# TomasDelaney/A-Deep-Reinforcement-Learning-Enabled-Soft-Exoskeleton-for-Parkinson-s-Patients

Measured on AMD Instinct MI355X. Metric: env steps/sec (batched exo sim) + TD7 grad-steps/sec at 1/2/4/8 MI355X, higher is better.
Workload: dtype f64 sim + bf16 TD7

## Files before the change

### a-deep-reinforcement-learning-enabled-soft-exoskeleton-for-parkinson-s-patients_amd/csrc/lap.hip

```cpp
#include <hip/hip_runtime.h>

#include <algorithm>
#include <cstdint>
#include <cstdlib>
#include <string>

#include "philox.h"
#include "exo_amd.h"

namespace {

constexpr int UPD_THREADS = 1024;

__device__ __forceinline__ float *stratum_tree(float *tree, int s, int cap) { return tree + (size_t)s * 2 * cap; }

constexpr int TOPN = 8192;
template <int NTOP = TOPN>
__device__ bool propagate_top(float *T, int cap, int levels, const int32_t *slot, int n, float *top) {
    int lv = 1;
    for (; lv <= levels && ((2 * cap) >> lv) > NTOP / 2; ++lv) {
        __syncthreads();
        for (int k = threadIdx.x; k < n; k += blockDim.x) {
            const int node = (cap + slot[k]) >> lv;
            T[node] = T[2 * node] + T[2 * node + 1];
        }
    }
    __syncthreads();
    if (lv > levels) return false;
    const int lim = min(NTOP, 2 * cap);
    if (blockDim.x == UPD_THREADS) {
        constexpr int PER = NTOP / UPD_THREADS;
        float v[PER];
#pragma unroll
        for (int j = 0; j < PER; ++j) {
            const int i = threadIdx.x + j * UPD_THREADS;
            v[j] = i < lim ? T[i] : 0.0f;
        }
#pragma unroll
        for (int j = 0; j < PER; ++j) {
            const int i = threadIdx.x + j * UPD_THREADS;
            if (i < lim) top[i] = v[j];
        }
    } else {
        for (int i = threadIdx.x; i < lim; i += blockDim.x) top[i] = T[i];
    }
    for (; lv <= levels; ++lv) {
        __syncthreads();
        for (int k = threadIdx.x; k < n; k += blockDim.x) {
            const int node = (cap + slot[k]) >> lv;
            top[node] = top[2 * node] + top[2 * node + 1];
        }
    }
    __syncthreads();
    const int wb = min(NTOP / 2, cap);
    for (int i = 1 + threadIdx.x; i < wb; i += blockDim.x) T[i] = top[i];
    __syncthreads();
    return true;
}
__device__ void propagate(float *T, int cap, int levels, const int32_t *slot, int n) {
    __shared__ float top[TOPN];
    propagate_top(T, cap, levels, slot, n, top);
}

__device__ void propagate_span(float *T, int cap, int levels, int capacity, int first, int count) {
    __shared__ float top[TOPN];
    if (count <= 0) return;
    int a0 = first, e0 = first + count, a1 = 0, e1 = 0;
    if (count >= capacity) {
        a0 = 0;
        e0 = capacity;
    } else if (e0 > capacity) {
        e1 = e0 - capacity;
        e0 = capacity;
    }
    int lv = 1;
    for (; lv <= levels && ((2 * cap) >> lv) > TOPN / 2; ++lv) {
        __syncthreads();
        const int lo0 = (cap + a0) >> lv, n0 = ((cap + e0 - 1) >> lv) - lo0 + 1;
        const int lo1 = (cap + a1) >> lv, n1 = e1 > a1 ? ((cap + e1 - 1) >> lv) - lo1 + 1 : 0;
        for (int k = threadIdx.x; k < n0 + n1; k += blockDim.x) {
            const int node = k < n0 ? lo0 + k : lo1 + k - n0;
            T[node] = T[2 * node] + T[2 * node + 1];
        }
    }
    __syncthreads();
    if (lv > levels) return;
    const int lim = min(TOPN, 2 * cap);
    for (int i = threadIdx.x; i < lim; i += blockDim.x) top[i] = T[i];
    for (; lv <= levels; ++lv) {
        __syncthreads();
        const int lo0 = (cap + a0) >> lv, n0 = ((cap + e0 - 1) >> lv) - lo0 + 1;
        const int lo1 = (cap + a1) >> lv, n1 = e1 > a1 ? ((cap + e1 - 1) >> lv) - lo1 + 1 : 0;
        for (int k = threadIdx.x; k < n0 + n1; k += blockDim.x) {
            const int node = k < n0 ? lo0 + k : lo1 + k - n0;
            top[node] = top[2 * node] + top[2 * node + 1];
        }
    }
    __syncthreads();
    const int wb = min(TOPN / 2, cap);
    for (int i = 1 + threadIdx.x; i < wb; i += blockDim.x) T[i] = top[i];
    __syncthreads();
}

constexpr int SPAN_LDS = 4096;
constexpr int SPAN_LEVELS = 32;
__device__ bool propagate_span_lds(float *T, int cap, int levels, int capacity, int first, int count,
                                   float *buf , float *edge ) {
    const int a = cap + first, e = cap + first + count - 1;
    if (count <= 0 || first + count > capacity || count > SPAN_LDS - 2 || levels >= SPAN_LEVELS) return false;
    const int t = threadIdx.x;
    if (t < 2 * levels) {
        const int lv = t >> 1, right = t & 1;
        const int lo = a >> lv, hi = e >> lv;
        if (!right && (lo & 1)) edge[t] = T[lo - 1];
        if (right && !(hi & 1)) edge[t] = T[hi + 1];
    }
    float *A = buf, *B = buf + SPAN_LDS;
    {
        const int base = a & ~1;
        for (int c = a + t; c <= e; c += blockDim.x) A[c - base] = T[c];
    }
    __syncthreads();
    if (t == 0) {
        if (a & 1) A[0] = edge[0];
        if (!(e & 1)) A[(e | 1) - (a & ~1)] = edge[1];
    }
    for (int lv = 1; lv <= levels; ++lv) {
        __syncthreads();
        const int lo = a >> lv, hi = e >> lv, cbase = (a >> (lv - 1)) & ~1, nbase = lo & ~1;
        for (int node = lo + t; node <= hi; node += blockDim.x) {
            const int c = 2 * node - cbase;
            const float v = A[c] + A[c + 1];
            T[node] = v;
            B[node - nbase] = v;
        }
        if (t == 0 && lv < levels) {
            if (lo & 1) B[0] = edge[2 * lv];
            if (!(hi & 1)) B[(hi | 1) - nbase] = edge[2 * lv + 1];
        }
        float *tmp = A;
        A = B;
        B = tmp;
    }
    __syncthreads();
    return true;
}

constexpr int ADD_CHUNK = 4096;
__global__ __launch_bounds__(UPD_THREADS) void lap_add_kernel(float *tree, const float *maxp, int cap, int levels,
                                                              int capacity, const int32_t *stratum,
                                                              const int32_t *slot, int n) {
    const int s = blockIdx.x;
    float *T = stratum_tree(tree, s, cap);
    __shared__ int32_t mine[ADD_CHUNK];
    __shared__ int count;
    const float p = *maxp;
    for (int base = 0; base < n; base += ADD_CHUNK) {
        if (threadIdx.x == 0) count = 0;
        __syncthreads();
// ... 845 lines not shown
}

__global__ __launch_bounds__(256) void lap_ref_plan_slots_kernel(int32_t *plan, long long entries,
                                                                 const int32_t *add_s, long long total,
                                                                 const long long *ref, int E, int capacity) {
    const long long i = (long long)blockIdx.x * blockDim.x + threadIdx.x;
    if (i >= entries) return;
    const int c = plan[i];
    if (c < 0) return;
    const long long ptr0 = ref[0], count0 = ref[1];
    const long long m0 = mult_below(count0, E), mr = mult_below(count0 + c, E);
    const long long qend = min(mr * E - count0, total - 1);
    const int s = add_s[c];
    bool win = true;
    for (long long q = c + 1; q <= qend; ++q) win &= add_s[q] != s;
    long long v = ptr0 + (mr - m0);
    if (v >= capacity) v -= capacity;
    if (v >= capacity) v %= capacity;
    plan[i] = win ? (int32_t)v : -1;
}

__global__ __launch_bounds__(256) void lap_ref_step_kernel(lap_storage_desc st, const int32_t *plan, int rows, int n,
                                                           long long *kk, int par, long long *k_dev,
                                                           const int32_t *strata, int capacity, const float *state,
                                                           const float *action, const float *next_state,
                                                           const float *reward, const uint8_t *done,
                                                           float action_scale, const uint8_t *table,
                                                           uint8_t *active, int32_t *count,
                                                           const int32_t *counts_table, double *score) {
    const long long k = kk[par];
    const long long k1 = k + 1 < rows ? k + 1 : rows - 1;
    const int e = blockIdx.x * 4 + (threadIdx.x >> 6), lane = threadIdx.x & 63;
    if (blockIdx.x == 0 && threadIdx.x == 0) {
        kk[par ^ 1] = k1;
        if (k_dev) *k_dev = k1;
        if (count) *count = counts_table[k1];
    }
    if (e >= n) return;
    const int slot = k < rows ? plan[(size_t)k * n + e] : -1;
    if (slot >= 0) {
        const long r = (long)strata[e] * (capacity + 1) + slot;
        const int sd = st.state_dim, ad = st.action_dim;
        for (int q = lane; q < sd; q += 64) {
            st.state[r * sd + q] = state[(long)e * sd + q];
            st.next_state[r * sd + q] = next_state[(long)e * sd + q];
        }
        for (int q = lane; q < ad; q += 64) st.action[r * ad + q] = action[(long)e * ad + q] / action_scale;
        if (lane == 0) {
            st.reward[r] = reward[e];
            st.not_done[r] = 1.0f - (done[e] ? 1.0f : 0.0f);
        }
    }
    if (lane == 0) {
        if (score) score[e] += active[e] ? (double)reward[e] : 0.0;
        active[e] = table[(size_t)k1 * n + e];
    }
}

__global__ __launch_bounds__(256) void lap_ref_commit_leaves_kernel(const int32_t *plan, long long entries, int n,
                                                                    const int32_t *strata, float *tree, int cap,
                                                                    const float *maxp) {
    const long long i = (long long)blockIdx.x * blockDim.x + threadIdx.x;
    if (i >= entries) return;
    const int slot = plan[i];
    if (slot < 0) return;
    stratum_tree(tree, strata[i % n], cap)[cap + slot] = *maxp;
}

__global__ __launch_bounds__(UPD_THREADS) void lap_ref_commit_tree_kernel(float *tree, int cap, int levels,
                                                                          int capacity, const long long *ref,
                                                                          long long total, int E) {
    const long long ptr0 = ref[0], count0 = ref[1];
    if (total <= 0) return;
    const long long last = mult_below(count0 + total - 1, E) - mult_below(count0, E);
    propagate_span(stratum_tree(tree, blockIdx.x, cap), cap, levels, capacity, (int)ptr0,
                   (int)min(last + 1, (long long)capacity));
}

__global__ void lap_ref_commit_ref_kernel(long long *ref, long long total, int E, int capacity, int32_t *ring_size) {
    const long long ptr0 = ref[0], count0 = ref[1], size0 = ref[2];
    const long long adv = mult_below(count0 + total, E) - mult_below(count0, E);
    const long long size = min(size0 + adv, (long long)capacity);
    for (int s = 0; s < E; ++s) ring_size[s] = (int32_t)size;
    ref[0] = (ptr0 + adv) % capacity;
    ref[1] = count0 + total;
    ref[2] = size;
}

constexpr int GATHER_DRAWS = 16;
__global__ __launch_bounds__(256) void lap_gather_kernel(lap_storage_desc st, int capacity, const int32_t *idx,
                                                         int batch, int total, float *o_state, float *o_action,
                                                         float *o_next, float *o_reward, float *o_not_done) {
    const int sd = st.state_dim, ad = st.action_dim;
    const bool v4 = (sd & 3) == 0 && ((reinterpret_cast<uintptr_t>(st.state) | reinterpret_cast<uintptr_t>(st.next_state) |
                                       reinterpret_cast<uintptr_t>(o_state) | reinterpret_cast<uintptr_t>(o_next)) & 15) == 0;
    const int sv = v4 ? sd / 4 : sd, per = 2 * sv + ad + 2;
    const int d0 = blockIdx.x * GATHER_DRAWS;
    const int nd = min(GATHER_DRAWS, total - d0);
    const int items = nd * per;
    constexpr int GU = 4;
    for (int it0 = threadIdx.x; it0 < items; it0 += GU * 256) {
        float4 v[GU];
        float *dst[GU];
        bool wide[GU];
#pragma unroll
        for (int u = 0; u < GU; ++u) {
            const int it = it0 + u * 256;
            dst[u] = nullptr;
            wide[u] = false;
            if (it >= items) continue;
            const int q = it / per, c = it - q * per;
            const long d = d0 + q;
            const long row = (long)(d / batch) * (capacity + 1) + idx[d];
            if (c < 2 * sv) {
                const bool nx = c >= sv;
                const int e = nx ? c - sv : c;
                const float *src = (nx ? st.next_state : st.state) + row * sd;
                float *o = (nx ? o_next : o_state) + d * sd;
                if (v4) {
                    v[u] = ld4(src + 4 * e);
                    dst[u] = o + 4 * e;
                    wide[u] = true;
                } else {
                    v[u].x = src[e];
                    dst[u] = o + e;
                }
            } else if (c < 2 * sv + ad) {
                const int e = c - 2 * sv;
                v[u].x = st.action[row * ad + e];
                dst[u] = o_action + d * ad + e;
            } else if (c == 2 * sv + ad) {
                v[u].x = st.reward[row];
                dst[u] = o_reward + d;
            } else {
                v[u].x = st.not_done[row];
                dst[u] = o_not_done + d;
            }
        }
#pragma unroll
        for (int u = 0; u < GU; ++u) {
            if (!dst[u]) continue;
            if (wide[u]) st4(dst[u], v[u]);
            else *dst[u] = v[u].x;
        }
    }
}

struct TdPrio {
    const float *td;
    float alpha, minp;
    float *out;
};

__global__ __launch_bounds__(UPD_THREADS) void lap_update_sample_kernel(float *tree, float *maxp, int cap, int levels,
                                                                        int capacity, const int32_t *idx_in,
                                                                        const float *prio, int batch,
                                                                        const int32_t *size, lap_storage_desc st,
                                                                        SampleRng rng, int32_t *idx_out,
                                                                        float *o_state, float *o_action, float *o_next,
                                                                        float *o_reward, float *o_not_done,
                                                                        TdPrio tp, bool gather) {
    const int s = blockIdx.x;
    float *T = stratum_tree(tree, s, cap);
    const int32_t *I = idx_in + (size_t)s * batch;
    const float *P = prio + (size_t)s * batch;
    __shared__ float red[UPD_THREADS / 64];
    __shared__ int32_t li[UPD_THREADS];
    __shared__ float top[TOPN_US];
    __shared__ int32_t pick[UPD_THREADS];
    const unsigned long long call = *rng.counter;
    float mx = 0.0f;
    for (int b0 = 0; b0 < batch; b0 += UPD_THREADS) {
        const int nb = min(UPD_THREADS, batch - b0);
        __syncthreads();
        if ((int)threadIdx.x < nb) li[threadIdx.x] = I[b0 + threadIdx.x];
        __syncthreads();
        const int b = b0 + threadIdx.x;
        if (b < batch) {
            const int me = li[threadIdx.x];
            bool last = true;
            for (int k = threadIdx.x + 1; k < nb; ++k) last &= (li[k] != me);
            for (int b2 = b0 + nb; b2 < batch; ++b2) last &= (I[b2] != me);
            float pb;
            if (tp.td) {
                const long d = (long)s * batch + b;
                pb = powf(fmaxf(fmaxf(tp.td[2 * d], tp.td[2 * d + 1]), tp.minp), tp.alpha);
                if (tp.out) tp.out[d] = pb;
            } else {
                pb = P[b];
            }
            if (last) T[cap + me] = pb;
            mx = fmaxf(mx, pb);
        }
    }
    for (int o = 32; o > 0; o >>= 1) mx = fmaxf(mx, __shfl_xor(mx, o, 64));
    if ((threadIdx.x & 63) == 0) red[threadIdx.x >> 6] = mx;
    const bool staged = propagate_top<TOPN_US>(T, cap, levels, I, batch, top);
    if (threadIdx.x == 0) {
        for (int w = 1; w < (int)(blockDim.x >> 6); ++w) mx = fmaxf(mx, red[w]);
        atomicMax(reinterpret_cast<int *>(maxp), __float_as_int(mx));
    }
    const int lim = staged ? min(TOPN_US, 2 * cap) : 0;
    auto node_at = [&](int node) { return node < lim ? top[node] : T[node]; };
    const int sz = size[s];
    const float tot = prefix_sum(node_at, cap, levels, sz);
    for (int b = threadIdx.x; b < batch; b += UPD_THREADS) {
        const int d = s * batch + b;
        uint32_t r[4];
        philox_block(rng.seed, rng.tag, call, (uint32_t)d, r);
        float val = u01_open_hi(r[0]) * tot;
        int node = 1, lv = 0;
        for (; lv < levels && 2 * node + 1 < lim; ++lv) {
            const float left = top[2 * node], right = top[2 * node + 1];
            if (val <= left || right <= 0.0f) {
                node = 2 * node;
            } else {
                val -= left;
                node = 2 * node + 1;
            }
        }
        node = descend_from([T](int n) { return T[n]; }, val, node, lv, levels);
        int i = node - cap;
        if (i >= sz) i = sz > 0 ? sz - 1 : 0;
        idx_out[d] = i;
        if (b < UPD_THREADS) pick[b] = i;
    }
    __syncthreads();
    if (!gather) {
        if (threadIdx.x == 0 && atomicAdd(rng.ticket, 1u) == gridDim.x - 1) {
            *rng.counter = call + 1ull;
            *rng.ticket = 0u;
        }
        return;
    }
    const int sd = st.state_dim, ad = st.action_dim;
    const bool v4 = (sd & 3) == 0 && ((reinterpret_cast<uintptr_t>(st.state) | reinterpret_cast<uintptr_t>(st.next_state) |
                                       reinterpret_cast<uintptr_t>(o_state) | reinterpret_cast<uintptr_t>(o_next)) & 15) == 0;
    const int sv = v4 ? sd / 4 : sd, per = 2 * sv + ad + 2;
    const int items = min(batch, UPD_THREADS) * per;
    constexpr int GU = 8;
    for (int it0 = threadIdx.x; it0 < items; it0 += GU * UPD_THREADS) {
        float4 v[GU];
        float *dst[GU];
        bool wide[GU];
#pragma unroll
        for (int u = 0; u < GU; ++u) {
            const int it = it0 + u * UPD_THREADS;
            dst[u] = nullptr;
            wide[u] = false;
            if (it >= items) continue;
            const int b = it / per, c = it - b * per;
            const long d = (long)s * batch + b;
            const long row = (long)s * (capacity + 1) + pick[b];
            if (c < 2 * sv) {
                const bool nx = c >= sv;
                const int e = nx ? c - sv : c;
                const float *src = (nx ? st.next_state : st.state) + row * sd;
                float *o = (nx ? o_next : o_state) + d * sd;
                if (v4) {
                    v[u] = ld4(src + 4 * e);
                    dst[u] = o + 4 * e;
                    wide[u] = true;
                } else {
                    v[u].x = src[e];
                    dst[u] = o + e;
                }
            } else if (c < 2 * sv + ad) {
                const int e = c - 2 * sv;
                v[u].x = st.action[row * ad + e];
                dst[u] = o_action + d * ad + e;
            } else if (c == 2 * sv + ad) {
                v[u].x = st.reward[row];
                dst[u] = o_reward + d;
            } else {
                v[u].x = st.not_done[row];
                dst[u] = o_not_done + d;
            }
        }
#pragma unroll
        for (int u = 0; u < GU; ++u) {
            if (!dst[u]) continue;
            if (wide[u]) st4(dst[u], v[u]);
            else *dst[u] = v[u].x;
        }
    }
    __syncthreads();
    if (threadIdx.x == 0) {
        if (atomicAdd(rng.ticket, 1u) == gridDim.x - 1) {
            *rng.counter = call + 1ull;
            *rng.ticket = 0u;
        }
    }
}

int rc(hipError_t e) { return e == hipSuccess ? EXO_OK : EXO_EDEVICE; }

int levels_of(const lap_tree_desc *t) {
    int lv = 0;
    while ((1 << lv) < t->cap) ++lv;
    return lv;
}

bool gather_split() {
    static const bool on = [] {
        const char *e = getenv("EXO_LAP_GATHER_SPLIT");
        return !(e && e[0] == '0');
    }();
    return on;
}

int gather_after(const lap_tree_desc *t, const lap_storage_desc *st, int batch, const int32_t *idx, float *o_state,
                 float *o_action, float *o_next, float *o_reward, float *o_not_done, void *stream) {
    if (hipGetLastError() != hipSuccess) return EXO_EDEVICE;
    if (!gather_split()) return EXO_OK;
    const int total = t->n_strata * batch;
    hipLaunchKernelGGL(lap_gather_kernel, dim3((total + GATHER_DRAWS - 1) / GATHER_DRAWS), dim3(256), 0,
                       (hipStream_t)stream, *st, t->capacity, idx, batch, total, o_state, o_action, o_next, o_reward,
                       o_not_done);
    return hipGetLastError() == hipSuccess ? EXO_OK : EXO_EDEVICE;
}

bool valid(const lap_tree_desc *t) {
    return t && t->tree && t->max_priority && t->n_strata > 0 && t->capacity > 0 && t->cap >= t->capacity &&
           (t->cap & (t->cap - 1)) == 0 && t->cap <= (1 << MAXLV);
}

}

extern "C" {

int32_t lap_tree_floats(int32_t n_strata, int32_t capacity) {
    int cap = 1;
    while (cap < capacity) cap <<= 1;
    return n_strata * 2 * cap;
}

int lap_init(const lap_tree_desc *t, void *stream) {
    if (!valid(t)) return EXO_EINVAL;
    hipError_t e = hipMemsetAsync(t->tree, 0, (size_t)t->n_strata * 2 * t->cap * sizeof(float), (hipStream_t)stream);
    if (e != hipSuccess) return EXO_EDEVICE;
    hipLaunchKernelGGL(lap_init_kernel, dim3(1), dim3(1), 0, (hipStream_t)stream, t->max_priority);
    return rc(hipGetLastError());
}

int lap_add(const lap_tree_desc *t, const int32_t *stratum, const int32_t *slot, int32_t n, void *stream) {
    if (!valid(t) || !stratum || !slot || n < 0) return EXO_EINVAL;
    if (n == 0) return EXO_OK;
    hipLaunchKernelGGL(lap_add_kernel, dim3(t->n_strata), dim3(UPD_THREADS), 0, (hipStream_t)stream, t->tree,
                       t->max_priority, t->cap, levels_of(t), t->capacity, stratum, slot, n);
    return rc(hipGetLastError());
}

int lap_sample(const lap_tree_desc *t, const float *u, const int32_t *size, int32_t batch, int32_t *idx, void *stream) {
    if (!valid(t) || !u || !size || !idx || batch <= 0) return EXO_EINVAL;
    const int th = 128;
    hipLaunchKernelGGL(lap_sample_kernel, dim3((batch + th - 1) / th, t->n_strata), dim3(th), 0, (hipStream_t)stream,
                       t->tree, t->cap, levels_of(t), u, size, batch, idx);
    return rc(hipGetLastError());
}

int lap_update(const lap_tree_desc *t, const int32_t *idx, const float *prio, int32_t batch, void *stream) {
    if (!valid(t) || !idx || !prio || batch <= 0) return EXO_EINVAL;
    hipLaunchKernelGGL(lap_update_kernel, dim3(t->n_strata), dim3(UPD_THREADS), 0, (hipStream_t)stream, t->tree,
                       t->max_priority, t->cap, levels_of(t), idx, prio, batch);
    return rc(hipGetLastError());
}

int lap_reset_max(const lap_tree_desc *t, void *stream) {
    if (!valid(t)) return EXO_EINVAL;
    hipError_t e = hipMemsetAsync(t->max_priority, 0, sizeof(float), (hipStream_t)stream);
    if (e != hipSuccess) return EXO_EDEVICE;
    hipLaunchKernelGGL(lap_reset_max_kernel, dim3(256), dim3(1024), 0, (hipStream_t)stream, t->tree, t->max_priority,
                       t->cap, t->n_strata);
    return rc(hipGetLastError());
}

int lap_totals(const lap_tree_desc *t, float *out, void *stream) {
    if (!valid(t) || !out) return EXO_EINVAL;
    hipLaunchKernelGGL(lap_totals_kernel, dim3((t->n_strata + 63) / 64), dim3(64), 0, (hipStream_t)stream, t->tree,
                       t->cap, t->n_strata, out);
    return rc(hipGetLastError());
}

int lap_store_batch(const lap_tree_desc *t, const lap_storage_desc *st, const float *state, const float *action,
                    const float *next_state, const float *reward, const uint8_t *done, const int32_t *strata,
                    const uint8_t *active, float action_scale, int32_t n, int32_t *row_ws, void *stream) {
    if (!valid(t) || !st || !st->state || !st->action || !st->next_state || !st->reward || !st->not_done ||
        !st->ptr || !st->size || st->state_dim <= 0 || st->action_dim <= 0 || !state || !action || !next_state ||
        !reward || !done || !strata || !row_ws || n < 0 || action_scale == 0.0f)
        return EXO_EINVAL;
    if (n == 0) return EXO_OK;
    const char *fused_var = getenv("EXO_LAP_STORE_FUSED");
    const bool fused_env = fused_var && fused_var[0] == '1';
    if (fused_env && n <= STORE_FUSED_MAX && n <= t->capacity) {
        const bool vec = (st->state_dim & 3) == 0 &&
                         ((reinterpret_cast<uintptr_t>(state) | reinterpret_cast<uintptr_t>(next_state) |
                           reinterpret_cast<uintptr_t>(st->state) | reinterpret_cast<uintptr_t>(st->next_state)) &
                          15) == 0;
        if (vec)
            hipLaunchKernelGGL(lap_store_fused_kernel<true>, dim3(t->n_strata), dim3(UPD_THREADS), 0,
                               (hipStream_t)stream, t->tree, t->max_priority, t->cap, levels_of(t), t->capacity,
                               st->ptr, st->size, strata, active, n, row_ws, *st, state, action, next_state, reward,
                               done, action_scale);
        else
            hipLaunchKernelGGL(lap_store_fused_kernel<false>, dim3(t->n_strata), dim3(UPD_THREADS), 0,
                               (hipStream_t)stream, t->tree, t->max_priority, t->cap, levels_of(t), t->capacity,
                               st->ptr, st->size, strata, active, n, row_ws, *st, state, action, next_state, reward,
                               done, action_scale);
        return rc(hipGetLastError());
    }
    if (n > 4 * STORE_CHUNK)
        hipLaunchKernelGGL(lap_store_rank_kernel<16>, dim3(t->n_strata), dim3(UPD_THREADS), 0, (hipStream_t)stream,
                           t->tree, t->max_priority, t->cap, levels_of(t), t->capacity, st->ptr, st->size, strata,
                           active, n, row_ws);
    else
        hipLaunchKernelGGL(lap_store_rank_kernel<4>, dim3(t->n_strata), dim3(UPD_THREADS), 0, (hipStream_t)stream,
                           t->tree, t->max_priority, t->cap, levels_of(t), t->capacity, st->ptr, st->size, strata,
                           active, n, row_ws);
    if (hipGetLastError() != hipSuccess) return EXO_EDEVICE;
    hipLaunchKernelGGL(lap_store_copy_kernel, dim3((n + 3) / 4), dim3(256), 0, (hipStream_t)stream, *st, state,
                       action, next_state, reward, done, action_scale, n, row_ws);
    return rc(hipGetLastError());
}

int lap_store_batch_ref(const lap_tree_desc *t, const lap_storage_desc *st, int64_t *ref_dev, const float *state,
                        const float *action, const float *next_state, const float *reward, const uint8_t *done,
                        const int32_t *strata, const uint8_t *active, float action_scale, int32_t n,
                        int32_t *ws_dev, void *stream) {
    if (!valid(t) || !st || !st->state || !st->action || !st->next_state || !st->reward || !st->not_done ||
        !st->size || st->state_dim <= 0 || st->action_dim <= 0 || !ref_dev || !state || !action || !next_state ||
        !reward || !done || !strata || !ws_dev || n < 0 || action_scale == 0.0f)
        return EXO_EINVAL;
    if (n == 0) return EXO_OK;
    int32_t *rank_row = ws_dev, *slot_of = ws_dev + n, *row_of = ws_dev + 2 * n;
    hipLaunchKernelGGL(lap_store_ref_slots_kernel, dim3(1), dim3(UPD_THREADS), 0, (hipStream_t)stream, t->capacity,
                       t->n_strata, (long long *)ref_dev, st->size, strata, active, n, rank_row, slot_of, row_of);
    if (hipGetLastError() != hipSuccess) return EXO_EDEVICE;
    hipLaunchKernelGGL(lap_add_kernel, dim3(t->n_strata), dim3(UPD_THREADS), 0, (hipStream_t)stream, t->tree,
                       t->max_priority, t->cap, levels_of(t), t->capacity, strata, slot_of, n);
    if (hipGetLastError() != hipSuccess) return EXO_EDEVICE;
    hipLaunchKernelGGL(lap_store_copy_kernel, dim3((n + 3) / 4), dim3(256), 0, (hipStream_t)stream, *st, state,
                       action, next_state, reward, done, action_scale, n, row_of);
    return rc(hipGetLastError());
}

static int store_ref_fused(const lap_tree_desc *t, const lap_storage_desc *st, int64_t *ref_dev,
                           const float *state, const float *action, const float *next_state, const float *reward,
                           const uint8_t *done, const int32_t *strata, const uint8_t *active, float action_scale,
                           int32_t n, uint32_t *ticket_dev, const MaskAdvance &adv, void *stream) {
    if (!valid(t) || !st || !st->state || !st->action || !st->next_state || !st->reward || !st->not_done ||
        !st->size || st->state_dim <= 0 || st->action_dim <= 0 || !ref_dev || !state || !action || !next_state ||
        !reward || !done || !strata || !ticket_dev || n < 0 || action_scale == 0.0f)
        return EXO_EINVAL;
    if (n == 0) return EXO_OK;
    const int E = t->n_strata;
    const int K = 1 + std::max(1, std::min(15, (n + E * 64 - 1) / (E * 64)));
    auto al16 = [](const void *p) { return ((uintptr_t)p & 15u) == 0; };
    const bool vec = st->state_dim % 4 == 0 && al16(state) && al16(next_state) && al16(st->state) &&
                     al16(st->next_state);
    if (vec)
        hipLaunchKernelGGL(lap_store_ref_fused_kernel<true>, dim3(E, K), dim3(UPD_THREADS), 0, (hipStream_t)stream,
                           t->tree, t->max_priority, t->cap, levels_of(t), t->capacity, E, (long long *)ref_dev,
                           st->size, *st, state, action, next_state, reward, done, action_scale, strata, active, n,
                           ticket_dev, adv);
    else
        hipLaunchKernelGGL(lap_store_ref_fused_kernel<false>, dim3(E, K), dim3(UPD_THREADS), 0, (hipStream_t)stream,
                           t->tree, t->max_priority, t->cap, levels_of(t), t->capacity, E, (long long *)ref_dev,
                           st->size, *st, state, action, next_state, reward, done, action_scale, strata, active, n,
                           ticket_dev, adv);
    return rc(hipGetLastError());
}

int lap_store_batch_ref_fused(const lap_tree_desc *t, const lap_storage_desc *st, int64_t *ref_dev,
                              const float *state, const float *action, const float *next_state, const float *reward,
                              const uint8_t *done, const int32_t *strata, const uint8_t *active, float action_scale,
                              int32_t n, uint32_t *ticket_dev, void *stream) {
    return store_ref_fused(t, st, ref_dev, state, action, next_state, reward, done, strata, active, action_scale, n,
                           ticket_dev, MaskAdvance{}, stream);
}

int lap_store_batch_ref_fused_adv(const lap_tree_desc *t, const lap_storage_desc *st, int64_t *ref_dev,
                                  const float *state, const float *action, const float *next_state,
                                  const float *reward, const uint8_t *done, const int32_t *strata, uint8_t *active,
                                  float action_scale, int32_t n, uint32_t *ticket_dev, const uint8_t *table,
                                  int32_t rows, int64_t *k_dev, int32_t *count_dev, double *score_dev, void *stream) {
    if (!table || rows <= 0 || !k_dev || !active) return EXO_EINVAL;
    return store_ref_fused(t, st, ref_dev, state, action, next_state, reward, done, strata, active, action_scale, n,
                           ticket_dev, MaskAdvance{table, rows, (long long *)k_dev, active, count_dev, score_dev},
                           stream);
}

int lap_sample_gather(const lap_tree_desc *t, const lap_storage_desc *st, const float *u, int32_t batch,
                      int32_t *idx, float *out_state, float *out_action, float *out_next_state, float *out_reward,
                      float *out_not_done, void *stream) {
    if (!valid(t) || !st || !st->size || !u || !idx || batch <= 0 || !out_state || !out_action ||
        !out_next_state || !out_reward || !out_not_done)
        return EXO_EINVAL;
    const int total = t->n_strata * batch;
    hipLaunchKernelGGL(lap_sample_gather_kernel, dim3((total + 3) / 4), dim3(256), 0, (hipStream_t)stream, t->tree,
                       t->cap, levels_of(t), t->capacity, u, st->size, batch, total, idx, *st, out_state, out_action,
                       out_next_state, out_reward, out_not_done, SampleRng{0, 0, nullptr, nullptr});
    return rc(hipGetLastError());
}

int lap_update_sample_rng(const lap_tree_desc *t, const lap_storage_desc *st, const int32_t *idx_in,
                          const float *prio, int32_t batch, uint64_t seed, uint32_t tag, unsigned long long *counter,
                          uint32_t *ticket, int32_t *idx_out, float *out_state, float *out_action,
                          float *out_next_state, float *out_reward, float *out_not_done, void *stream) {
    if (!valid(t) || !st || !st->size || !idx_in || !prio || !counter || !ticket || !idx_out || batch <= 0 ||
        batch > UPD_THREADS || !out_state || !out_action || !out_next_state || !out_reward || !out_not_done)
        return EXO_EINVAL;
    hipLaunchKernelGGL(lap_update_sample_kernel, dim3(t->n_strata), dim3(UPD_THREADS), 0, (hipStream_t)stream,
                       t->tree, t->max_priority, t->cap, levels_of(t), t->capacity, idx_in, prio, batch, st->size,
                       *st, SampleRng{seed, tag, counter, ticket}, idx_out, out_state, out_action, out_next_state,
                       out_reward, out_not_done, TdPrio{nullptr, 0.f, 0.f, nullptr}, !gather_split());
    return gather_after(t, st, batch, idx_out, out_state, out_action, out_next_state, out_reward, out_not_done, stream);
}

int lap_update_sample_idx(const lap_tree_desc *t, const lap_storage_desc *st, const int32_t *idx_in,
                          const float *prio, int32_t batch, uint64_t seed, uint32_t tag, unsigned long long *counter,
                          uint32_t *ticket, int32_t *idx_out, void *stream) {
    if (!valid(t) || !st || !st->size || !idx_in || !prio || !counter || !ticket || !idx_out || batch <= 0 ||
        batch > UPD_THREADS)
        return EXO_EINVAL;
    hipLaunchKernelGGL(lap_update_sample_kernel, dim3(t->n_strata), dim3(UPD_THREADS), 0, (hipStream_t)stream,
                       t->tree, t->max_priority, t->cap, levels_of(t), t->capacity, idx_in, prio, batch, st->size,
                       *st, SampleRng{seed, tag, counter, ticket}, idx_out, nullptr, nullptr, nullptr, nullptr,
                       nullptr, TdPrio{nullptr, 0.f, 0.f, nullptr}, false);
    return rc(hipGetLastError());
}

int lap_gather_rows(const lap_tree_desc *t, const lap_storage_desc *st, int32_t batch, const int32_t *idx,
                    float *out_state, float *out_action, float *out_next_state, float *out_reward,
                    float *out_not_done, void *stream) {
    if (!valid(t) || !st || !st->state || !st->action || !st->next_state || !st->reward || !st->not_done || !idx ||
        batch <= 0 || !out_state || !out_action || !out_next_state || !out_reward || !out_not_done)
        return EXO_EINVAL;
    const int total = t->n_strata * batch;
    hipLaunchKernelGGL(lap_gather_kernel, dim3((total + GATHER_DRAWS - 1) / GATHER_DRAWS), dim3(256), 0,
                       (hipStream_t)stream, *st, t->capacity, idx, batch, total, out_state, out_action,
                       out_next_state, out_reward, out_not_done);
    return rc(hipGetLastError());
}

int lap_update_sample_td(const lap_tree_desc *t, const lap_storage_desc *st, const int32_t *idx_in, const float *td,
                         float alpha, float min_priority, float *prio_out, int32_t batch, uint64_t seed, uint32_t tag,
                         unsigned long long *counter, uint32_t *ticket, int32_t *idx_out, float *out_state,
                         float *out_action, float *out_next_state, float *out_reward, float *out_not_done,
                         void *stream) {
    if (!valid(t) || !st || !st->size || !idx_in || !td || !counter || !ticket || !idx_out || batch <= 0 ||
        batch > UPD_THREADS || !out_state || !out_action || !out_next_state || !out_reward || !out_not_done)
        return EXO_EINVAL;
    hipLaunchKernelGGL(lap_update_sample_kernel, dim3(t->n_strata), dim3(UPD_THREADS), 0, (hipStream_t)stream,
                       t->tree, t->max_priority, t->cap, levels_of(t), t->capacity, idx_in, (const float *)nullptr,
                       batch, st->size, *st, SampleRng{seed, tag, counter, ticket}, idx_out, out_state, out_action,
                       out_next_state, out_reward, out_not_done, TdPrio{td, alpha, min_priority, prio_out},
                       !gather_split());
    return gather_after(t, st, batch, idx_out, out_state, out_action, out_next_state, out_reward, out_not_done, stream);
}

int lap_sample_gather_rng(const lap_tree_desc *t, const lap_storage_desc *st, uint64_t seed, uint32_t tag,
                          unsigned long long *counter, uint32_t *ticket, int32_t batch, int32_t *idx,
                          float *out_state, float *out_action, float *out_next_state, float *out_reward,
                          float *out_not_done, void *stream) {
    if (!valid(t) || !st || !st->size || !counter || !ticket || !idx || batch <= 0 || !out_state || !out_action ||
        !out_next_state || !out_reward || !out_not_done)
        return EXO_EINVAL;
    const int total = t->n_strata * batch;
    hipLaunchKernelGGL(lap_sample_gather_kernel, dim3((total + 3) / 4), dim3(256), 0, (hipStream_t)stream, t->tree,
                       t->cap, levels_of(t), t->capacity, nullptr, st->size, batch, total, idx, *st, out_state,
                       out_action, out_next_state, out_reward, out_not_done, SampleRng{seed, tag, counter, ticket});
    return rc(hipGetLastError());
}


int lap_ref_plan(const lap_tree_desc *t, const int64_t *ref_dev, const uint8_t *table_dev, int32_t rows, int32_t n,
                 const int32_t *strata_dev, const int64_t *offs_dev, int64_t total, int32_t *add_ws_dev,
                 int32_t *plan_dev, void *stream) {
    if (!valid(t) || !ref_dev || !table_dev || rows <= 0 || n <= 0 || !strata_dev || !offs_dev || total < 0 ||
        (total > 0 && !add_ws_dev) || !plan_dev)
        return EXO_EINVAL;
    hipStream_t s = (hipStream_t)stream;
    hipLaunchKernelGGL(lap_ref_plan_scan_kernel, dim3(rows), dim3(UPD_THREADS), 0, s, table_dev, n, strata_dev,
                       t->n_strata, (const long long *)offs_dev, add_ws_dev, plan_dev);
    if (hipGetLastError() != hipSuccess) return EXO_EDEVICE;
    const long long entries = (long long)rows * n;
    hipLaunchKernelGGL(lap_ref_plan_slots_kernel, dim3((unsigned)((entries + 255) / 256)), dim3(256), 0, s, plan_dev,
                       entries, add_ws_dev, (long long)total, (const long long *)ref_dev, t->n_strata, t->capacity);
    return rc(hipGetLastError());
}

int lap_ref_step(const lap_tree_desc *t, const lap_storage_desc *st, const int32_t *plan_dev, int32_t rows,
                 int32_t n, int64_t *kk_dev, int32_t par, int64_t *k_dev, const int32_t *strata_dev,
                 const float *state, const float *action, const float *next_state, const float *reward,
                 const uint8_t *done, float action_scale, const uint8_t *table_dev, uint8_t *active_dev,
                 int32_t *count_dev, const int32_t *counts_table_dev, double *score_dev, void *stream) {
    if (!valid(t) || !st || !st->state || !st->action || !st->next_state || !st->reward || !st->not_done ||
        !plan_dev || rows <= 0 || n <= 0 || !kk_dev || (par != 0 && par != 1) || !strata_dev || !state || !action ||
        !next_state || !reward || !done || action_scale == 0.0f || !table_dev || !active_dev ||
        (count_dev && !counts_table_dev))
        return EXO_EINVAL;
    hipLaunchKernelGGL(lap_ref_step_kernel, dim3((n + 3) / 4), dim3(256), 0, (hipStream_t)stream, *st, plan_dev,
                       rows, n, (long long *)kk_dev, par, (long long *)k_dev, strata_dev, t->capacity, state, action,
                       next_state, reward, done, action_scale, table_dev, active_dev, count_dev, counts_table_dev,
                       score_dev);
    return rc(hipGetLastError());
}

int lap_ref_commit(const lap_tree_desc *t, const lap_storage_desc *st, int64_t *ref_dev, const int32_t *plan_dev,
                   int32_t rows, int32_t n, const int32_t *strata_dev, int64_t total, void *stream) {
    if (!valid(t) || !st || !st->size || !ref_dev || !plan_dev || rows <= 0 || n <= 0 || !strata_dev || total < 0)
        return EXO_EINVAL;
    hipStream_t s = (hipStream_t)stream;
    const long long entries = (long long)rows * n;
    hipLaunchKernelGGL(lap_ref_commit_leaves_kernel, dim3((unsigned)((entries + 255) / 256)), dim3(256), 0, s,
                       plan_dev, entries, n, strata_dev, t->tree, t->cap, t->max_priority);
    hipLaunchKernelGGL(lap_ref_commit_tree_kernel, dim3(t->n_strata), dim3(UPD_THREADS), 0, s, t->tree, t->cap,
                       levels_of(t), t->capacity, (const long long *)ref_dev, (long long)total, t->n_strata);
    hipLaunchKernelGGL(lap_ref_commit_ref_kernel, dim3(1), dim3(1), 0, s, (long long *)ref_dev, (long long)total,
                       t->n_strata, t->capacity, st->size);
    return rc(hipGetLastError());
}

}
```

Baseline: 17.09 million.

## Add chained sum-tree update kernel for small batches in LAP update-sample

Adds a new update-and-sample kernel used when batch is at most 256. It finds, for each updated leaf, which other updated leaf shares its subtree at each level (the partner) and detects duplicate slots by pairwise comparison. Each thread then walks its own leaf-to-root chain, reading partner sums from LDS instead of running level-synchronous global propagation passes. Loads, RNG draws and staging of the top of the tree are overlapped before the first barrier, and raw s_waitcnt+s_barrier replaces __syncthreads. It can be disabled with EXO_LAP_CHAIN=0, but the per-launch getenv call and the more complex chain logic add overhead and correctness risk.

Measured after the change: 17.34 million (median of 6 runs). No clear change (+1.4%).

```diff
diff --git a/a-deep-reinforcement-learning-enabled-soft-exoskeleton-for-parkinson-s-patients_amd/csrc/lap.hip b/a-deep-reinforcement-learning-enabled-soft-exoskeleton-for-parkinson-s-patients_amd/csrc/lap.hip
--- a/a-deep-reinforcement-learning-enabled-soft-exoskeleton-for-parkinson-s-patients_amd/csrc/lap.hip
+++ b/a-deep-reinforcement-learning-enabled-soft-exoskeleton-for-parkinson-s-patients_amd/csrc/lap.hip
@@ -5,6 +5,7 @@
 #include <cstdlib>
 #include <string>
 
+#include "lap_chain.h"
 #include "philox.h"
 #include "exo_amd.h"
 
@@ -1156,87 +1157,9 @@
     float *out;
 };
 
-__global__ __launch_bounds__(UPD_THREADS) void lap_update_sample_kernel(float *tree, float *maxp, int cap, int levels,
-                                                                        int capacity, const int32_t *idx_in,
-                                                                        const float *prio, int batch,
-                                                                        const int32_t *size, lap_storage_desc st,
-                                                                        SampleRng rng, int32_t *idx_out,
-                                                                        float *o_state, float *o_action, float *o_next,
-                                                                        float *o_reward, float *o_not_done,
-                                                                        TdPrio tp, bool gather) {
-    const int s = blockIdx.x;
-    float *T = stratum_tree(tree, s, cap);
-    const int32_t *I = idx_in + (size_t)s * batch;
-    const float *P = prio + (size_t)s * batch;
-    __shared__ float red[UPD_THREADS / 64];
-    __shared__ int32_t li[UPD_THREADS];
-    __shared__ float top[TOPN_US];
-    __shared__ int32_t pick[UPD_THREADS];
-    const unsigned long long call = *rng.counter;
-    float mx = 0.0f;
-    for (int b0 = 0; b0 < batch; b0 += UPD_THREADS) {
-        const int nb = min(UPD_THREADS, batch - b0);
-        __syncthreads();
-        if ((int)threadIdx.x < nb) li[threadIdx.x] = I[b0 + threadIdx.x];
-        __syncthreads();
-        const int b = b0 + threadIdx.x;
-        if (b < batch) {
-            const int me = li[threadIdx.x];
-            bool last = true;
-            for (int k = threadIdx.x + 1; k < nb; ++k) last &= (li[k] != me);
-            for (int b2 = b0 + nb; b2 < batch; ++b2) last &= (I[b2] != me);
-            float pb;
-            if (tp.td) {
-                const long d = (long)s * batch + b;
-                pb = powf(fmaxf(fmaxf(tp.td[2 * d], tp.td[2 * d + 1]), tp.minp), tp.alpha);
-                if (tp.out) tp.out[d] = pb;
-            } else {
-                pb = P[b];
-            }
-            if (last) T[cap + me] = pb;
-            mx = fmaxf(mx, pb);
-        }
-    }
-    for (int o = 32; o > 0; o >>= 1) mx = fmaxf(mx, __shfl_xor(mx, o, 64));
-    if ((threadIdx.x & 63) == 0) red[threadIdx.x >> 6] = mx;
-    const bool staged = propagate_top<TOPN_US>(T, cap, levels, I, batch, top);
-    if (threadIdx.x == 0) {
-        for (int w = 1; w < (int)(blockDim.x >> 6); ++w) mx = fmaxf(mx, red[w]);
-        atomicMax(reinterpret_cast<int *>(maxp), __float_as_int(mx));
-    }
-    const int lim = staged ? min(TOPN_US, 2 * cap) : 0;
-    auto node_at = [&](int node) { return node < lim ? top[node] : T[node]; };
-    const int sz = size[s];
-    const float tot = prefix_sum(node_at, cap, levels, sz);
-    for (int b = threadIdx.x; b < batch; b += UPD_THREADS) {
-        const int d = s * batch + b;
-        uint32_t r[4];
-        philox_block(rng.seed, rng.tag, call, (uint32_t)d, r);
-        float val = u01_open_hi(r[0]) * tot;
-        int node = 1, lv = 0;
-        for (; lv < levels && 2 * node + 1 < lim; ++lv) {
-            const float left = top[2 * node], right = top[2 * node + 1];
-            if (val <= left || right <= 0.0f) {
-                node = 2 * node;
-            } else {
-                val -= left;
-                node = 2 * node + 1;
-            }
-        }
-        node = descend_from([T](int n) { return T[n]; }, val, node, lv, levels);
-        int i = node - cap;
-        if (i >= sz) i = sz > 0 ? sz - 1 : 0;
-        idx_out[d] = i;
-        if (b < UPD_THREADS) pick[b] = i;
-    }
-    __syncthreads();
-    if (!gather) {
-        if (threadIdx.x == 0 && atomicAdd(rng.ticket, 1u) == gridDim.x - 1) {
-            *rng.counter = call + 1ull;
-            *rng.ticket = 0u;
-        }
-        return;
-    }
+__device__ __forceinline__ void gather_picked(const lap_storage_desc &st, int capacity, int s, int batch,
+                                              const int32_t *pick, float *o_state, float *o_action, float *o_next,
+                                              float *o_reward, float *o_not_done) {
     const int sd = st.state_dim, ad = st.action_dim;
     const bool v4 = (sd & 3) == 0 && ((reinterpret_cast<uintptr_t>(st.state) | reinterpret_cast<uintptr_t>(st.next_state) |
                                        reinterpret_cast<uintptr_t>(o_state) | reinterpret_cast<uintptr_t>(o_next)) & 15) == 0;
@@ -1288,12 +1211,278 @@
             else *dst[u] = v[u].x;
         }
     }
+}
+
+__global__ __launch_bounds__(UPD_THREADS) void lap_update_sample_kernel(float *tree, float *maxp, int cap, int levels,
+                                                                        int capacity, const int32_t *idx_in,
+                                                                        const float *prio, int batch,
+                                                                        const int32_t *size, lap_storage_desc st,
+                                                                        SampleRng rng, int32_t *idx_out,
+                                                                        float *o_state, float *o_action, float *o_next,
+                                                                        float *o_reward, float *o_not_done,
+                                                                        TdPrio tp, bool gather) {
+    const int s = blockIdx.x;
+    float *T = stratum_tree(tree, s, cap);
+    const int32_t *I = idx_in + (size_t)s * batch;
+    const float *P = prio + (size_t)s * batch;
+    __shared__ float red[UPD_THREADS / 64];
+    __shared__ int32_t li[UPD_THREADS];
+    __shared__ float top[TOPN_US];
+    __shared__ int32_t pick[UPD_THREADS];
+    const unsigned long long call = *rng.counter;
+    float mx = 0.0f;
+    for (int b0 = 0; b0 < batch; b0 += UPD_THREADS) {
+        const int nb = min(UPD_THREADS, batch - b0);
+        __syncthreads();
+        if ((int)threadIdx.x < nb) li[threadIdx.x] = I[b0 + threadIdx.x];
+        __syncthreads();
+        const int b = b0 + threadIdx.x;
+        if (b < batch) {
+            const int me = li[threadIdx.x];
+            bool last = true;
+            for (int k = threadIdx.x + 1; k < nb; ++k) last &= (li[k] != me);
+            for (int b2 = b0 + nb; b2 < batch; ++b2) last &= (I[b2] != me);
+            float pb;
+            if (tp.td) {
+                const long d = (long)s * batch + b;
+                pb = powf(fmaxf(fmaxf(tp.td[2 * d], tp.td[2 * d + 1]), tp.minp), tp.alpha);
+                if (tp.out) tp.out[d] = pb;
+            } else {
+                pb = P[b];
+            }
+            if (last) T[cap + me] = pb;
+            mx = fmaxf(mx, pb);
+        }
+    }
+    for (int o = 32; o > 0; o >>= 1) mx = fmaxf(mx, __shfl_xor(mx, o, 64));
+    if ((threadIdx.x & 63) == 0) red[threadIdx.x >> 6] = mx;
+    const bool staged = propagate_top<TOPN_US>(T, cap, levels, I, batch, top);
+    if (threadIdx.x == 0) {
+        for (int w = 1; w < (int)(blockDim.x >> 6); ++w) mx = fmaxf(mx, red[w]);
+        atomicMax(reinterpret_cast<int *>(maxp), __float_as_int(mx));
+    }
+    const int lim = staged ? min(TOPN_US, 2 * cap) : 0;
+    auto node_at = [&](int node) { return node < lim ? top[node] : T[node]; };
+    const int sz = size[s];
+    const float tot = prefix_sum(node_at, cap, levels, sz);
+    for (int b = threadIdx.x; b < batch; b += UPD_THREADS) {
+        const int d = s * batch + b;
+        uint32_t r[4];
+        philox_block(rng.seed, rng.tag, call, (uint32_t)d, r);
+        float val = u01_open_hi(r[0]) * tot;
+        int node = 1, lv = 0;
+        for (; lv < levels && 2 * node + 1 < lim; ++lv) {
+            const float left = top[2 * node], right = top[2 * node + 1];
+            if (val <= left || right <= 0.0f) {
+                node = 2 * node;
+            } else {
+                val -= left;
+                node = 2 * node + 1;
+            }
+        }
+        node = descend_from([T](int n) { return T[n]; }, val, node, lv, levels);
+        int i = node - cap;
+        if (i >= sz) i = sz > 0 ? sz - 1 : 0;
+        idx_out[d] = i;
+        if (b < UPD_THREADS) pick[b] = i;
+    }
+    __syncthreads();
+    if (!gather) {
+        if (threadIdx.x == 0 && atomicAdd(rng.ticket, 1u) == gridDim.x - 1) {
+            *rng.counter = call + 1ull;
+            *rng.ticket = 0u;
+        }
+        return;
+    }
+    gather_picked(st, capacity, s, batch, pick, o_state, o_action, o_next, o_reward, o_not_done);
     __syncthreads();
     if (threadIdx.x == 0) {
         if (atomicAdd(rng.ticket, 1u) == gridDim.x - 1) {
             *rng.counter = call + 1ull;
             *rng.ticket = 0u;
         }
+    }
+}
+
+constexpr int CHAIN_MAXB = 256;
+constexpr int CHAIN_MAXG = 12;
+constexpr int CHAIN_ROW = CHAIN_MAXB + 1;
+constexpr int CHAIN_TOPLV = 12;
+static_assert((2 << CHAIN_TOPLV) >= TOPN_US, "CHAIN_TOPLV: the staged top's levels");
+constexpr int CHAIN_PAD = 0x40000000;
+constexpr int CHAIN_RNG0 = 640;
+
+__device__ __forceinline__ void lds_barrier() { asm volatile("s_waitcnt lgkmcnt(0)\n\ts_barrier" ::: "memory"); }
+
+__global__ __launch_bounds__(UPD_THREADS) void lap_update_sample_chain_kernel(
+    float *tree, float *maxp, int cap, int levels, int capacity, const int32_t *idx_in,
+    const float *__restrict__ prio, int batch, const int32_t *__restrict__ size, lap_storage_desc st, SampleRng rng,
+    int32_t *idx_out, float *o_state, float *o_action, float *o_next, float *o_reward, float *o_not_done, TdPrio tp,
+    bool gather) {
+    const int s = blockIdx.x, t = threadIdx.x;
+    float *T = stratum_tree(tree, s, cap);
+    __shared__ float red[UPD_THREADS / 64];
+    __shared__ __attribute__((aligned(16))) int32_t li[CHAIN_MAXB + 4];
+    __shared__ int32_t lsz;
+    __shared__ float uni[CHAIN_MAXB];
+    __shared__ int32_t later[CHAIN_MAXB];
+    __shared__ int32_t partner[CHAIN_MAXG * CHAIN_ROW];
+    __shared__ float chain[2][CHAIN_MAXB];
+    __shared__ float lowval[CHAIN_MAXG];
+    __shared__ float top[TOPN_US];
+    __shared__ int32_t pick[CHAIN_MAXB];
+    const int G = lap_chain::global_levels(levels, TOPN_US);
+    const int lim = min(TOPN_US, 2 * cap);
+    const bool draw = t < batch;
+    const long d = (long)s * batch + (draw ? t : 0);
+    const unsigned long long call = *rng.counter;
+    const int sz = size[s];
+    const int me = idx_in[d];
+    const float *pp = tp.td ? tp.td + 2 * d : prio + d;
+    const float p0 = pp[0], p1 = pp[tp.td ? 1 : 0];
+    constexpr int PER = TOPN_US / UPD_THREADS;
+    float stage[PER];
+#pragma unroll
+    for (int j = 0; j < PER; ++j) stage[j] = T[min(t + j * UPD_THREADS, lim - 1)];
+    for (int i = t; i < G * CHAIN_ROW; i += UPD_THREADS) partner[i] = -1;
+    if (t < CHAIN_MAXB + 4) li[t] = draw ? me : CHAIN_PAD;
+    if (draw) later[t] = 0;
+    if (t >= CHAIN_RNG0 && t < CHAIN_RNG0 + batch) {
+        uint32_t r[4];
+        philox_block(rng.seed, rng.tag, call, (uint32_t)(s * batch + t - CHAIN_RNG0), r);
+        uni[t - CHAIN_RNG0] = u01_open_hi(r[0]);
+    }
+    const int szl = min(sz, cap - 1);
+    const int leaf = t == batch ? szl : me;
+    if (t == batch) lsz = szl;
+    float sib[CHAIN_MAXG];
+#pragma unroll
+    for (int lv = 0; lv < CHAIN_MAXG; ++lv) sib[lv] = 0.0f;
+    if (t <= batch) {
+#pragma unroll
+        for (int lv = 0; lv < CHAIN_MAXG; ++lv) sib[lv] = T[lap_chain::sibling_of(cap, leaf, min(lv, max(G - 1, 0)))];
+    }
+    lds_barrier();
+    {
+        int lp = 0;
+        while (((batch + 1) << (lp + 1)) <= UPD_THREADS) ++lp;
+        const int b = t >> lp, part = t & ((1 << lp) - 1);
+        const int chunk = (((batch + 3) >> 2) + (1 << lp) - 1) >> lp;
+        if (b <= batch) {
+            const int mine = b < batch ? li[b] : lsz;
+            const unsigned near = 1u << G;
+            bool sup = false;
+            for (int q = part * chunk; q < (part + 1) * chunk && 4 * q < batch; ++q) {
+                const int4 o = *reinterpret_cast<const int4 *>(&li[4 * q]);
+                const int other[4] = {o.x, o.y, o.z, o.w};
+#pragma unroll
+                for (int j = 0; j < 4; ++j) {
+                    const int k = 4 * q + j;
+                    if ((unsigned)(mine ^ other[j]) >= near) continue;
+                    const int lv = lap_chain::partner_level(mine, other[j]);
+                    if (lv < 0) sup |= b < batch && lap_chain::superseded_by(b, mine, k, other[j]);
+                    else atomicMax(&partner[lv * CHAIN_ROW + b], k);
+                }
+            }
+            if (sup) later[b] = 1;
+        }
+    }
+    const float pb = !draw ? 0.0f : tp.td ? powf(fmaxf(fmaxf(p0, p1), tp.minp), tp.alpha) : p0;
+    float mx = pb;
+    for (int o = 32; o > 0; o >>= 1) mx = fmaxf(mx, __shfl_xor(mx, o, 64));
+    if ((t & 63) == 0) red[t >> 6] = mx;
+#pragma unroll
+    for (int j = 0; j < PER; ++j) {
+        const int i = t + j * UPD_THREADS;
+        if (i < lim) top[i] = stage[j];
+    }
+    lds_barrier();
+    const bool carry = draw && !later[t];
+    if (draw && tp.td && tp.out) tp.out[d] = pb;
+    float cur = pb;
+    if (carry) {
+        T[cap + me] = pb;
+        chain[0][t] = pb;
+    }
+    if (t == batch) {
+#pragma unroll
+        for (int lv = 0; lv < CHAIN_MAXG; ++lv)
+            if (lv < G && partner[lv * CHAIN_ROW + batch] < 0) lowval[lv] = sib[lv];
+    }
+#pragma unroll
+    for (int lv = 0; lv < CHAIN_MAXG; ++lv) {
+        if (lv < G) lds_barrier();
+        if (lv < G && carry) {
+            if (partner[lv * CHAIN_ROW + batch] == t) lowval[lv] = cur;
+            const int node = lap_chain::node_of(cap, me, lv), k = partner[lv * CHAIN_ROW + t];
+            cur = lap_chain::chain_step(node, cur, k >= 0 ? chain[lv & 1][k] : sib[lv]);
+            T[node >> 1] = cur;
+            chain[(lv + 1) & 1][t] = cur;
+        }
+    }
+    if (carry) top[lap_chain::node_of(cap, me, G)] = cur;
+    for (int lv = G + 1; lv <= levels; ++lv) {
+        lds_barrier();
+        if (draw) {
+            const int node = lap_chain::node_of(cap, me, lv);
+            top[node] = top[2 * node] + top[2 * node + 1];
+        }
+    }
+    __syncthreads();
+    const int wb = min(TOPN_US / 2, cap);
+    for (int i = 1 + t; i < wb; i += UPD_THREADS) T[i] = top[i];
+    if (t >= UPD_THREADS - 64) {
+        float m = red[t & (UPD_THREADS / 64 - 1)];
+        for (int o = UPD_THREADS / 128; o > 0; o >>= 1) m = fmaxf(m, __shfl_xor(m, o, 64));
+        if (t == UPD_THREADS - 64) atomicMax(reinterpret_cast<int *>(maxp), __float_as_int(m));
+    }
+    if (draw) {
+        const int ltop = levels - G;
+        float tot;
+        if (sz >= cap) {
+            tot = top[1];
+        } else {
+            float x[CHAIN_TOPLV];
+#pragma unroll
+            for (int j = 0; j < CHAIN_TOPLV; ++j) {
+                const int lv = levels - 1 - j;
+                x[j] = j < ltop ? top[2 * ((1 << j) | (sz >> (lv + 1)))] : 0.0f;
+            }
+            tot = 0.0f;
+#pragma unroll
+            for (int j = 0; j < CHAIN_TOPLV; ++j)
+                if (j < ltop) tot += ((sz >> (levels - 1 - j)) & 1) ? x[j] : 0.0f;
+#pragma unroll
+            for (int lv = CHAIN_MAXG - 1; lv >= 0; --lv) {
+                if (lv >= G) continue;
+                tot += ((sz >> lv) & 1) ? lowval[lv] : 0.0f;
+            }
+        }
+        float val = uni[t] * tot;
+        int node = 1;
+        for (int lv = 0; lv < ltop; ++lv) {
+            const float left = top[2 * node], right = top[2 * node + 1];
+            if (val <= left || right <= 0.0f) {
+                node = 2 * node;
+            } else {
+                val -= left;
+                node = 2 * node + 1;
+            }
+        }
+        node = descend_from([T](int n) { return T[n]; }, val, node, ltop, levels);
+        int i = node - cap;
+        if (i >= sz) i = sz > 0 ? sz - 1 : 0;
+        idx_out[d] = i;
+        pick[t] = i;
+    }
+    __syncthreads();
+    if (gather) {
+        gather_picked(st, capacity, s, batch, pick, o_state, o_action, o_next, o_reward, o_not_done);
+        __syncthreads();
+    }
+    if (t == 0 && atomicAdd(rng.ticket, 1u) == gridDim.x - 1) {
+        *rng.counter = call + 1ull;
+        *rng.ticket = 0u;
     }
 }
 
@@ -1311,6 +1500,23 @@
         return !(e && e[0] == '0');
     }();
     return on;
+}
+
+void launch_update_sample(const lap_tree_desc *t, const lap_storage_desc *st, const int32_t *idx_in, const float *prio,
+                          int batch, SampleRng rng, int32_t *idx_out, float *o_state, float *o_action, float *o_next,
+                          float *o_reward, float *o_not_done, TdPrio tp, bool gather, void *stream) {
+    const char *e = getenv("EXO_LAP_CHAIN");
+    const int levels = levels_of(t);
+    const bool chain = !(e && e[0] == '0') && batch <= CHAIN_MAXB && levels >= 1 &&
+                       lap_chain::global_levels(levels, TOPN_US) <= CHAIN_MAXG;
+    if (chain)
+        hipLaunchKernelGGL(lap_update_sample_chain_kernel, dim3(t->n_strata), dim3(UPD_THREADS), 0, (hipStream_t)stream,
+                           t->tree, t->max_priority, t->cap, levels, t->capacity, idx_in, prio, batch, st->size, *st,
+                           rng, idx_out, o_state, o_action, o_next, o_reward, o_not_done, tp, gather);
+    else
+        hipLaunchKernelGGL(lap_update_sample_kernel, dim3(t->n_strata), dim3(UPD_THREADS), 0, (hipStream_t)stream,
+                           t->tree, t->max_priority, t->cap, levels, t->capacity, idx_in, prio, batch, st->size, *st,
+                           rng, idx_out, o_state, o_action, o_next, o_reward, o_not_done, tp, gather);
 }
 
 int gather_after(const lap_tree_desc *t, const lap_storage_desc *st, int batch, const int32_t *idx, float *o_state,
@@ -1514,10 +1720,9 @@
     if (!valid(t) || !st || !st->size || !idx_in || !prio || !counter || !ticket || !idx_out || batch <= 0 ||
         batch > UPD_THREADS || !out_state || !out_action || !out_next_state || !out_reward || !out_not_done)
         return EXO_EINVAL;
-    hipLaunchKernelGGL(lap_update_sample_kernel, dim3(t->n_strata), dim3(UPD_THREADS), 0, (hipStream_t)stream,
-                       t->tree, t->max_priority, t->cap, levels_of(t), t->capacity, idx_in, prio, batch, st->size,
-                       *st, SampleRng{seed, tag, counter, ticket}, idx_out, out_state, out_action, out_next_state,
-                       out_reward, out_not_done, TdPrio{nullptr, 0.f, 0.f, nullptr}, !gather_split());
+    launch_update_sample(t, st, idx_in, prio, batch, SampleRng{seed, tag, counter, ticket}, idx_out, out_state,
+                         out_action, out_next_state, out_reward, out_not_done, TdPrio{nullptr, 0.f, 0.f, nullptr},
+                         !gather_split(), stream);
     return gather_after(t, st, batch, idx_out, out_state, out_action, out_next_state, out_reward, out_not_done, stream);
 }
 
@@ -1527,10 +1732,8 @@
     if (!valid(t) || !st || !st->size || !idx_in || !prio || !counter || !ticket || !idx_out || batch <= 0 ||
         batch > UPD_THREADS)
         return EXO_EINVAL;
-    hipLaunchKernelGGL(lap_update_sample_kernel, dim3(t->n_strata), dim3(UPD_THREADS), 0, (hipStream_t)stream,
-                       t->tree, t->max_priority, t->cap, levels_of(t), t->capacity, idx_in, prio, batch, st->size,
-                       *st, SampleRng{seed, tag, counter, ticket}, idx_out, nullptr, nullptr, nullptr, nullptr,
-                       nullptr, TdPrio{nullptr, 0.f, 0.f, nullptr}, false);
+    launch_update_sample(t, st, idx_in, prio, batch, SampleRng{seed, tag, counter, ticket}, idx_out, nullptr, nullptr,
+                         nullptr, nullptr, nullptr, TdPrio{nullptr, 0.f, 0.f, nullptr}, false, stream);
     return rc(hipGetLastError());
 }
 
@@ -1555,11 +1758,9 @@
     if (!valid(t) || !st || !st->size || !idx_in || !td || !counter || !ticket || !idx_out || batch <= 0 ||
         batch > UPD_THREADS || !out_state || !out_action || !out_next_state || !out_reward || !out_not_done)
         return EXO_EINVAL;
-    hipLaunchKernelGGL(lap_update_sample_kernel, dim3(t->n_strata), dim3(UPD_THREADS), 0, (hipStream_t)stream,
-                       t->tree, t->max_priority, t->cap, levels_of(t), t->capacity, idx_in, (const float *)nullptr,
-                       batch, st->size, *st, SampleRng{seed, tag, counter, ticket}, idx_out, out_state, out_action,
-                       out_next_state, out_reward, out_not_done, TdPrio{td, alpha, min_priority, prio_out},
-                       !gather_split());
+    launch_update_sample(t, st, idx_in, nullptr, batch, SampleRng{seed, tag, counter, ticket}, idx_out, out_state,
+                         out_action, out_next_state, out_reward, out_not_done,
+                         TdPrio{td, alpha, min_priority, prio_out}, !gather_split(), stream);
     return gather_after(t, st, batch, idx_out, out_state, out_action, out_next_state, out_reward, out_not_done, stream);
 }
 
diff --git a/a-deep-reinforcement-learning-enabled-soft-exoskeleton-for-parkinson-s-patients_amd/csrc/lap_chain.h b/a-deep-reinforcement-learning-enabled-soft-exoskeleton-for-parkinson-s-patients_amd/csrc/lap_chain.h
--- /dev/null
+++ b/a-deep-reinforcement-learning-enabled-soft-exoskeleton-for-parkinson-s-patients_amd/csrc/lap_chain.h
@@ -0,0 +1,32 @@
+#pragma once
+
+#if defined(__HIPCC__)
+#define LAP_CHAIN_HD __host__ __device__ __forceinline__
+#else
+#define LAP_CHAIN_HD inline
+#endif
+
+namespace lap_chain {
+
+LAP_CHAIN_HD int global_levels(int levels, int ntop) {
+    int g = 0;
+    for (int lv = 1; lv <= levels; ++lv)
+        if (((2ll << levels) >> lv) > ntop / 2) ++g;
+    return g;
+}
+
+LAP_CHAIN_HD int node_of(int cap, int slot, int lv) { return (cap + slot) >> lv; }
+LAP_CHAIN_HD int sibling_of(int cap, int slot, int lv) { return node_of(cap, slot, lv) ^ 1; }
+
+LAP_CHAIN_HD int partner_level(int me, int other) {
+    const unsigned d = (unsigned)(me ^ other);
+    return d ? 31 - __builtin_clz(d) : -1;
+}
+
+LAP_CHAIN_HD bool superseded_by(int b, int me, int k, int other) { return k > b && other == me; }
+
+LAP_CHAIN_HD float chain_step(int node, float mine, float sibling) {
+    return (node & 1) ? sibling + mine : mine + sibling;
+}
+
+}
```
